# multimodallearning/stroke-prediction

Measured on AMD Instinct MI355X. Metric: train-step voxels/sec, 3D U-Net Bx2x128^3, higher is better.
Workload: dtype bf16; 1 GPU; configs[1]: U-Net 2 16 32 64 32 16 32 2, B=4/GPU, 2x128^3 -> 2x88^3, train_batch = fwd+Dice+bwd+Adam; global_batch=4, parallelism=dp1, launch=hipGraph (Learner(graph=True)), input=resident in the step's input buffers (Learner.static_batch)

## Files before the change

include/stroke_amd.h:

```cpp
#ifndef STROKE_AMD_H
#define STROKE_AMD_H

#include <stddef.h>
#include <stdint.h>

#ifdef __cplusplus
extern "C" {
#endif

typedef void* sp_stream_t;

enum { SP_OK = 0, SP_EINVAL = -1, SP_EHIP = -2 };
enum { SP_REDUCE_ROWS = 8 };
#define SP_DICE_PITCH(C) ((3 * (C) + 15) / 16 * 16)
enum { SP_VLOSS_DICE = 1, SP_VLOSS_BCE = 2 };
#define SP_VLOSS_PITCH(C) ((4 * (C) + 15) / 16 * 16)
#define SP_BLOSS_PITCH(C) SP_VLOSS_PITCH(C)
enum { SP_BF16 = 0, SP_F32 = 1,
       SP_HL = 2 };
enum { SP_ACT_NONE = 0, SP_ACT_LEAKY = 1, SP_ACT_ELU = 2, SP_ACT_SIGMOID = 3 };

int sp_version(void);
void sp_last_error(char* buf, size_t n);

typedef struct sp_bn_fin_args {
  const double* sums;
  const float* gamma;
  const float* beta;
  float* running_mean;
  float* running_var;
  float* scale;
  float* shift;
  float* mean;
  float* invstd;
  double count;
  float momentum, eps;
  int32_t nrep, training, C, CP;
} sp_bn_fin_args;

typedef struct sp_bn_bwd_args {
  const double* sums;
  const float* gamma;
  const float* mean;
  const float* invstd;
  float* dgamma;
  float* dbeta;
  float* coef;
  double count;
  float pscale;
  int32_t nrep, C, CP;
} sp_bn_bwd_args;

typedef struct sp_conv_args {
  const void* x;
  void* y;
  const void* wfrag_hi;
  const void* wfrag_lo;
  const float* in_scale;
  const float* in_shift;
  const float* bias;
  double* stats;
  const int32_t* ktab;
  int32_t dtype_in, dtype_out;
  int32_t B, Di, Hi, Wi, CPi;
  int32_t Do, Ho, Wo;
  int32_t YD, YH, YW, CPo;
  int32_t osD, osH, osW;
  int32_t ooD, ooH, ooW;
  int32_t Cout;
  int32_t sD, sH, sW;
  int32_t o0D, o0H, o0W;
  int32_t TD, TH;
  int32_t ITD, ITH, ITW;
  int32_t MT, NT;
  int32_t NTtot;
  int32_t ngroups;
  int32_t octs_per_group;
  int32_t opp;
  int32_t vsb;
  int32_t plane_bytes;
  int32_t lo_offset;
  int32_t steps_per_group;
  int32_t lds_bytes;
  int32_t act;
  float act_param;
  int32_t dma;
  int32_t zfill;
  int32_t persist;
  const void* aux;
  int32_t stats_mode;
  int32_t stats_nrep;
  int32_t ITH_zs;
  int64_t x_plane;
  void* y8;
  int64_t y8_plane;
  const float* f8_wscale;
  float y8_scale;
  int32_t f8_bin;
  int32_t group_batch;
  int32_t nslices;
  int64_t slice_wfrag_stride;
  int64_t x_lo_delta;
  int64_t y_lo_delta;
  const float* bias_tab;
  int32_t bias_tab_gstride;
  int32_t pad_;
  int64_t wfrag_gstride;
  sp_bn_bwd_args bnb;
  double* dz_sums;
  void* pool_y;
  int64_t pool_lo_delta;
  void* y2;
  int32_t split_nt, CPo2;
  int32_t pser_planes, pad2_;
} sp_conv_args;

int sp_conv3d_igemm(const sp_conv_args* a, sp_stream_t stream);
int sp_conv_prep_folded_groups(const float* w, int64_t sCo, int64_t sCi, int32_t Cout, int32_t Cin, const int32_t* kmap, int32_t nsteps,
                               int32_t NTtot, void* wfrag, int64_t frag_gstride, const float* coef, int32_t coef_gstride,
                               int32_t coef_pitch, int32_t G, const float* bias, int32_t padD, int32_t padH, int32_t padW,
                               float* bias_tab, int32_t CoutPad, sp_stream_t stream);
int sp_conv3d_igemm_multi(const sp_conv_args* args, int32_t n, sp_stream_t stream);
int sp_conv3d_par(const sp_conv_args* args, int32_t n, const void* gtab, const int32_t* gofs, const void* zeros, sp_stream_t stream);

int sp_conv3d_zm(const sp_conv_args* a, const void* zeros, sp_stream_t stream);
int sp_conv3d_zm_config(int32_t P, int32_t NT, int32_t* MT, int32_t* NSLOT, int32_t* NW);
int sp_conv3d_zm_config_ps(int32_t NT, int32_t hl, int32_t* MT, int32_t* NSLOT, int32_t* NW);

int sp_conv3d_zm_config_hl(int32_t P, int32_t NT, int32_t* MT, int32_t* NSLOT, int32_t* NW);
int sp_bn_stats_ncdhw_f32(const float* x, int32_t B, int32_t C, int64_t DHW, int32_t CP, double* sums, int32_t nrep,
                          sp_stream_t stream);
int sp_first_prep_hl(const float* w, const float* b, const float* scale, const float* shift, void* wfrag_hi, void* wfrag_lo,
                     float* bias_f, int32_t Cout, sp_stream_t stream);
int sp_first_conv_fwd_hl(const float* x, int32_t B, int32_t D, int32_t H, int32_t W, const void* wfrag_hi, const void* wfrag_lo,
                         const float* bias_f, int32_t act, float act_param, void* y, void* y_lo, double* stats, int32_t nrep,
                         int32_t Cout, sp_stream_t stream);
int sp_maxpool2_fwd_hl(const void* x, int64_t x_lo_delta, void* y, int64_t y_lo_delta, int32_t B, int32_t D, int32_t H, int32_t W,
                       int32_t CP, double* stats, sp_stream_t stream);
int sp_upsample2_crop_cat_fwd_hl(const void* low, int64_t low_lo_delta, int32_t CPu, const void* skip, int64_t skip_lo_delta, int32_t CPs,
                                 void* cat, int64_t cat_lo_delta, int32_t CPd, int32_t B, int32_t D, int32_t H, int32_t W, int32_t Ds,
                                 int32_t Hs, int32_t Ws, int64_t cat_plane, double* stats, sp_stream_t stream);
int sp_head_fwd_hl(const void* x, int64_t x_lo_delta, int64_t nvox_per_b, int32_t B, int32_t CP, int32_t C, const float* w1,
                   const float* b1, int32_t CH, const float* w2, const float* b2, int32_t NC, float slope, float* seg,
                   sp_stream_t stream);

int sp_conv3d_zm8(const sp_conv_args* a, const void* zeros, sp_stream_t stream);
int sp_conv_partial_finish(const float* partial, int32_t ngroups, int64_t nvox, int32_t CP, const float* bias ,
                           int32_t bias_stride, int32_t act, float act_param, void* y, double* stats ,
                           int32_t stats_nrep, void* y8 ,
                           int64_t y8_plane, sp_stream_t stream);
int sp_conv3d_zm8_config(int32_t P, int32_t NT, int32_t* MT, int32_t* NSLOT, int32_t* NW);
int sp_conv_prep_f8(const float* w, int64_t sCo, int64_t sCi, int32_t Cout, int32_t Cin, const int32_t* kmap,
                    int32_t nsteps, int32_t NT, void* wfrag, const float* fold_scale, const float* fold_shift,
                    int32_t ntaps, const float* bias, float* bias_out, float* winv, float out_scale, sp_stream_t stream);
typedef struct sp_f8_prep_item {
  const float* w;
  int64_t sCo, sCi;
  int32_t Cout, Cin;
  const int32_t* kmap;
  int32_t nsteps, NT;
  void* wfrag;
  const float* fold_scale;
  const float* fold_shift;
  const float* bias;
  float* bias_out;
  float* winv;
  int32_t ntaps;
  float out_scale;
} sp_f8_prep_item;
int sp_conv_prep_f8_batch(const sp_f8_prep_item* items_dev, int32_t n, int32_t max_rows, sp_stream_t stream);
int sp_quantize_f8(const void* src, int32_t CP, int64_t src_plane, void* dst, int64_t dst_plane, int64_t nvox, int32_t fmt,
                   float scale, sp_stream_t stream);

typedef struct sp_conv3d_desc {
  int32_t B, Cin, Cout, D, H, W;
  int32_t grad;
  int32_t padD, padH, padW;
  int32_t transposed;
} sp_conv3d_desc;
typedef struct sp_conv3d_plan_t {
  int32_t cin_op, cout_op;
  int32_t P, NT, MT, NW, NSLOT, KS, nsteps, ITH;
  int32_t Di, Hi, Wi, Do, Ho, Wo, o0;
  int32_t o0H, o0W, mirror;
  int64_t x_elems, y_elems;
  int64_t workspace_bytes;
  int64_t off_zero, off_ktab, off_kmap, off_bias, off_wfrag;
} sp_conv3d_plan_t;
int sp_conv3d_plan(const sp_conv3d_desc* d, sp_conv3d_plan_t* plan);
int sp_conv3d_tables(const sp_conv3d_desc* d, const sp_conv3d_plan_t* plan, int32_t* ktab, int32_t* kmap);
int sp_conv3d_init(const sp_conv3d_desc* d, const sp_conv3d_plan_t* plan, void* workspace, sp_stream_t stream);
int sp_conv3d_set_weights(const sp_conv3d_desc* d, const sp_conv3d_plan_t* plan, void* workspace, const float* w,
                          const float* bias, const float* bn_scale, const float* bn_shift, sp_stream_t stream);
int sp_conv3d_run(const sp_conv3d_desc* d, const sp_conv3d_plan_t* plan, const void* workspace, const void* x, void* y,
                  int32_t with_bias, int32_t act, float act_param, double* stats, int32_t stats_nrep, int64_t x_plane,
                  sp_stream_t stream);

typedef struct sp_conv3d_wgrad_plan_t {
  int32_t CoT, CiT, nblocks, Do, Ho, Wo;
  int64_t workspace_bytes, off_taps, off_tapsrc, off_acc;
} sp_conv3d_wgrad_plan_t;
int sp_conv3d_wgrad_plan(const sp_conv3d_desc* d, sp_conv3d_wgrad_plan_t* p);
int sp_conv3d_wgrad_init(const sp_conv3d_desc* d, const sp_conv3d_wgrad_plan_t* p, void* workspace, sp_stream_t stream);
int sp_conv3d_wgrad_run(const sp_conv3d_desc* d, const sp_conv3d_wgrad_plan_t* p, void* workspace, const void* x, const void* dz,
                        float* dw, const float* bn_scale , const float* bn_shift, const double* dbias_sums ,
                        int32_t dbias_stride, float* dbias_grad , const float* w_for_bn ,
                        double* bn_sums , int32_t bn_nrep, int64_t x_plane, sp_stream_t stream);

typedef struct sp_conv_fc_args {
  const void* x;
  void* y;
  const void* wfrag;
  const float* in_scale;
  const float* in_shift;
  const float* bias;
  double* stats;
  const void* aux;
  float* partial;
  const int32_t* taps;
  int32_t B, Di, Hi, Wi, CPi, Do, Ho, Wo, CPo, Cout;
  int32_t sD, sH, sW, o0D, o0H, o0W;
  int32_t ntap;
  int32_t act;
  float act_param;
  int32_t stats_mode, stats_nrep, dtype_out;
  int64_t x_plane;
  int32_t group_batch;
  int32_t coef_gstride;
} sp_conv_fc_args;
int sp_conv_fc_workspace(int32_t B, int32_t Do, int32_t Ho, int32_t Wo, int32_t Cout, int32_t ntap, int64_t* floats);
int sp_conv_fc(const sp_conv_fc_args* a, sp_stream_t stream);

int sp_conv_prep_weights(const float* w, int64_t sCo, int64_t sCi, int32_t Cout, int32_t Cin,
                         const int32_t* kmap, int32_t nsteps, int32_t NTtot,
                         void* wfrag_hi, void* wfrag_lo ,
                         const float* fold_scale ,
                         sp_stream_t stream);
typedef struct sp_prep_item {
  const float* w;
  int64_t sCo, sCi;
  int32_t Cout, Cin;
  const int32_t* kmap;
  int32_t nsteps, NTtot;
  void* wfrag_hi;
  void* wfrag_lo;
  const float* fold_scale;
  const float* bias;
  float* bias_out;
  int32_t bias_n, bias_pad;
} sp_prep_item;
int sp_conv_prep_weights_batch(const sp_prep_item* items_dev, int32_t n, int32_t max_blocks, sp_stream_t stream);
int sp_conv_fold_bias(const float* w, int64_t sCo, int64_t sCi, int32_t Cout, int32_t Cin, int32_t ntaps,
                      const float* bias, const float* shift, float* bias_out, int32_t CoutPad, sp_stream_t stream);
int sp_conv_prep_folded(const float* w, int64_t sCo, int64_t sCi, int32_t Cout, int32_t Cin, const int32_t* kmap,
                        int32_t nsteps, int32_t NTtot, void* wfrag_hi, void* wfrag_lo, const float* fold_scale,
                        int32_t ntaps, const float* bias, const float* fold_shift, float* bias_out, int32_t CoutPad,
                        sp_stream_t stream);

int sp_conv_prep_folded_bn(const float* w, int64_t sCo, int64_t sCi, int32_t Cout, int32_t Cin, const int32_t* kmap,
                           int32_t nsteps, int32_t NTtot, void* wfrag_hi, void* wfrag_lo, int32_t ntaps, const float* bias,
                           float* bias_out, int32_t CoutPad, const sp_bn_fin_args* bn, sp_stream_t stream);
int sp_first_prep_bn(const float* w, const float* b, void* wfrag, void* wfrag_lo, float* bias_f, int32_t Cout,
                     const sp_bn_fin_args* bn, sp_stream_t stream);

typedef struct sp_wgrad_args {
  const void* x;
  const void* dz;
  const float* in_scale;
  const float* in_shift;
  const float* dz_scale;
// ... 313 lines not shown
```

stroke-prediction_amd/csrc/sp_conv_dma.hip:

```cpp
#include "sp_common.h"

struct ConvDmaDev {
  sp_conv_args a;
  FastDiv d_itw, d_ith, d_plane;
  FastDiv d_tx, d_ty, d_tz;
  uint32_t ntx, nty, ntz, nblk;
  int32_t plane_chunks, group_chunks, nruns, log2_opp;
  int32_t row_chunks, segs_per_row, nrows, njobs;
  FastDiv d_segs, d_rows;
};

typedef __attribute__((address_space(3))) void lds_void;
typedef const __attribute__((address_space(1))) void gbl_void;


#ifdef SP_CONV_STAMPS
#define SP_NSTAMP 6
extern __device__ unsigned long long sp_stamp_buf[32768][SP_NSTAMP];
#define STAMP(k)                                                                              \
  do {                                                                                        \
    __builtin_amdgcn_sched_barrier(0);                                                        \
    unsigned long long t_;                                                                    \
    asm volatile("s_memtime %0\n\ts_waitcnt lgkmcnt(0)" : "=s"(t_)::"memory");                \
    __builtin_amdgcn_sched_barrier(0);                                                        \
    if (threadIdx.x == 0 && blockIdx.y == 0 && blockIdx.x < 32768) sp_stamp_buf[blockIdx.x][k] = t_; \
  } while (0)
#else
#define STAMP(k)
#endif

template <int NT, int MT, int KS, typename TOUT, bool HL = false>
__global__ __launch_bounds__(256, ((NT == 1 && KS > 0) ? 4 : 1)) void conv_igemm_dma_kernel(const ConvDmaDev P) {
  static_assert(!HL || KS == 0, "bf16 pairs: run-time K loop only");
  extern __shared__ __attribute__((aligned(16))) unsigned char lds[];
  const sp_conv_args& a = P.a;
  const int tid = threadIdx.x, lane = tid & 63, wave = __builtin_amdgcn_readfirstlane(tid >> 6);
  const int lv = lane & 15, lg = lane >> 4;

  uint32_t t = xcd_remap(blockIdx.x, P.nblk);
  uint32_t q = fdiv(t, P.d_tx); const int tx = t - q * P.ntx; t = q;
  q = fdiv(t, P.d_ty); const int ty = t - q * P.nty; t = q;
  q = fdiv(t, P.d_tz); const int tz = t - q * P.ntz; const int b = q;
  const int oz0 = tz * a.TD, oy0 = ty * a.TH, ox0 = tx * 16;
  const int nt0 = blockIdx.y * NT;
  const int iz0 = oz0 * a.sD + a.o0D, iy0 = oy0 * a.sH + a.o0H, ix0 = ox0 * a.sW + a.o0W;

  int* ktab_l = reinterpret_cast<int*>(lds);
  const int ktab_bytes = (a.steps_per_group * 16 + 15) & ~15;
  unsigned char* tile = lds + ktab_bytes;
  for (int i = tid; i < a.steps_per_group * 4; i += 256) ktab_l[i] = a.ktab[i];

  int vbase[MT];
#pragma unroll
  for (int m = 0; m < MT; ++m) {
    const int r = wave * MT + m;
    const int rz = r / a.TH, ry = r - rz * a.TH;
    vbase[m] = ((rz * a.sD * a.ITH + ry * a.sH) * a.ITW + lv * a.sW) * a.vsb;
  }
  f32x4 acc[NT][MT];
#pragma unroll
  for (int n = 0; n < NT; ++n)
#pragma unroll
    for (int m = 0; m < MT; ++m) acc[n][m] = f32x4{0.f, 0.f, 0.f, 0.f};

  const int xpitch = a.x_plane ? 16 : a.CPi;
  const bf16_t* __restrict__ xin = reinterpret_cast<const bf16_t*>(a.x) + (size_t)b * a.Di * a.Hi * a.Wi * xpitch;
  const bf16x8* __restrict__ wf_hi = reinterpret_cast<const bf16x8*>(a.wfrag_hi);
  const bool border = a.zfill && (iz0 < 0 || iy0 < 0 || ix0 < 0 || iz0 + a.ITD > a.Di || iy0 + a.ITH > a.Hi || ix0 + a.ITW > a.Wi);
  const int opp_mask = a.opp - 1;

  int job_goff[2], job_loff[2];
#pragma unroll
  for (int k = 0; k < 2; ++k) {
    int j = k * 64 + lane;
    j = j < P.njobs ? j : P.njobs - 1;
    const uint32_t prow = fdiv(j, P.d_segs);
    const int seg = j - prow * P.segs_per_row;
    const uint32_t pl = fdiv(prow, P.d_rows);
    const int row = prow - pl * P.nrows;
    const uint32_t vz = fdiv(row, P.d_ith);
    const int vy = row - vz * a.ITH;
    const int cz = min(max(iz0 + (int)vz, 0), a.Di - 1), cy = min(max(iy0 + vy, 0), a.Hi - 1);
    job_goff[k] = ((cz * a.Hi + cy) * a.Wi) * xpitch + (a.x_plane ? (int)pl * (int)a.x_plane : (int)pl * a.opp * 8);
    job_loff[k] = (int)pl * a.plane_bytes + row * P.row_chunks * 16 + seg * 1024 + (seg << 24);
  }
  STAMP(0);
  for (int grp = 0; grp < a.ngroups; ++grp) {
    if (grp > 0) __syncthreads();
    const int oct0 = grp * a.octs_per_group;
#pragma unroll
    for (int k = 0; k < 2; ++k) {
      const int nj = min(64, P.njobs - k * 64);
      for (int j = wave; j < nj; j += 4) {
        const int goff = __builtin_amdgcn_readlane(job_goff[k], j);
        const int lo = __builtin_amdgcn_readlane(job_loff[k], j);
        const int seg = lo >> 24;
        const int ch = seg * 64 + lane;
        if (ch < P.row_chunks) {
          const int cx = min(max(ix0 + (ch >> P.log2_opp), 0), a.Wi - 1);
          const bf16_t* src = a.x_plane ? xin + goff + (size_t)(oct0 >> 1) * a.x_plane + (cx * 16 + (ch & opp_mask) * 8)
                                        : xin + goff + (cx * a.CPi + (oct0 + (ch & opp_mask)) * 8);
#ifndef SP_NO_DMA
          sp_dma16(src, tile + (lo & 0xffffff));
          if constexpr (HL) sp_dma16(reinterpret_cast<const unsigned char*>(src) + a.x_lo_delta, tile + a.lo_offset + (lo & 0xffffff));
#endif
        }
      }
    }
    const size_t gstep0 = (size_t)grp * a.steps_per_group;
    const size_t fstride = (size_t)a.NTtot * 64;
    const bf16x8* wp = wf_hi + (gstep0 * a.NTtot + nt0) * 64 + lane;
    const bf16x8* wpl = HL ? reinterpret_cast<const bf16x8*>(a.wfrag_lo) + (gstep0 * a.NTtot + nt0) * 64 + lane : nullptr;
    bf16x8 wreg[KS > 0 ? KS : 1][NT];
    bf16x8 wa0[NT], wa1[NT];
    bf16x8 wl0[HL ? NT : 1], wl1[HL ? NT : 1], wl2[HL ? NT : 1], wl3[HL ? NT : 1];
    if (KS > 0) {
#pragma unroll
      for (int s = 0; s < KS; ++s)
#pragma unroll
        for (int n = 0; n < NT; ++n) wreg[s][n] = wp[s * fstride + (size_t)n * 64];
    } else {
#pragma unroll
      for (int n = 0; n < NT; ++n) wa0[n] = wp[(size_t)n * 64];
      if constexpr (HL) {
#pragma unroll
        for (int n = 0; n < NT; ++n) wl0[n] = wpl[(size_t)n * 64];
      }
    }
    if (grp == 0) STAMP(1);
    asm volatile("s_waitcnt vmcnt(0)" ::: "memory");
    __syncthreads();
    if (grp == 0) STAMP(2);
    if (border) {
      for (int r = wave; r < P.nruns; r += 4) {
        const int i = r * 64 + lane;
        if (i < P.group_chunks) {
          const uint32_t pl = fdiv(i, P.d_plane);
          const int ii = i - pl * P.plane_chunks;
          const uint32_t vox = (uint32_t)ii >> P.log2_opp;
          const uint32_t row = fdiv(vox, P.d_itw);
          const int vx = vox - row * a.ITW;
          const uint32_t vz = fdiv(row, P.d_ith);
          const int vy = row - vz * a.ITH;
          const int gz = iz0 + (int)vz, gy = iy0 + vy, gx = ix0 + vx;
          if (!((unsigned)gz < (unsigned)a.Di && (unsigned)gy < (unsigned)a.Hi && (unsigned)gx < (unsigned)a.Wi)) {
            *reinterpret_cast<uint4*>(tile + (size_t)i * 16) = make_uint4(0, 0, 0, 0);
            if constexpr (HL) *reinterpret_cast<uint4*>(tile + a.lo_offset + (size_t)i * 16) = make_uint4(0, 0, 0, 0);
          }
        }
      }
      __syncthreads();
    }

    bf16x8 x0[MT], x1[MT];
    bf16x8 xl0[HL ? MT : 1], xl1[HL ? MT : 1];
#define SP_LDX(dst, koff_)                                                                            \
  _Pragma("unroll") for (int m = 0; m < MT; ++m) dst[m] = *reinterpret_cast<const bf16x8*>(tile + vbase[m] + (koff_));
#define SP_LDXL(dst, koff_)                                                                           \
  if constexpr (HL) { _Pragma("unroll") for (int m = 0; m < MT; ++m) dst[m] = *reinterpret_cast<const bf16x8*>(tile + a.lo_offset + vbase[m] + (koff_)); }
#define SP_MMA(wv, xv)                                                                                \
  _Pragma("unroll") for (int m = 0; m < MT; ++m)                                                      \
      _Pragma("unroll") for (int n = 0; n < NT; ++n) acc[n][m] = SP_MFMA16(wv[n], xv[m], acc[n][m], 0, 0, 0);
#define SP_MMAL(wv, wlv, xv, xlv)                                                                     \
  if constexpr (HL) {                                                                                 \
    _Pragma("unroll") for (int m = 0; m < MT; ++m)                                                    \
        _Pragma("unroll") for (int n = 0; n < NT; ++n) {                                              \
          acc[n][m] = SP_MFMA16(wv[n], xlv[m], acc[n][m], 0, 0, 0);                                   \
          acc[n][m] = SP_MFMA16(wlv[n], xv[m], acc[n][m], 0, 0, 0);                                   \
        }                                                                                             \
  }
    {
      const int k0 = ktab_l[lg];
      SP_LDX(x0, k0)
      SP_LDXL(xl0, k0)
    }
    if (KS > 0) {
#pragma unroll
      for (int s = 0; s < KS; ++s) {
        if (s + 1 < KS) {
          const int kn = ktab_l[(s + 1) * 4 + lg];
          if ((s & 1) == 0) { SP_LDX(x1, kn) } else { SP_LDX(x0, kn) }
        }
        if ((s & 1) == 0) { SP_MMA(wreg[s], x0) } else { SP_MMA(wreg[s], x1) }
      }
    } else {
      const int nst = a.steps_per_group;
      bf16x8 wa2[NT], wa3[NT];
#define SP_LDW(dst, dstl, step_)                                                                      \
  { const int st_ = (step_) < nst ? (step_) : nst - 1;                                                \
    _Pragma("unroll") for (int n = 0; n < NT; ++n) dst[n] = wp[(size_t)st_ * fstride + (size_t)n * 64]; \
    if constexpr (HL) { _Pragma("unroll") for (int n = 0; n < NT; ++n) dstl[n] = wpl[(size_t)st_ * fstride + (size_t)n * 64]; } }
      SP_LDW(wa1, wl1, 1)
      SP_LDW(wa2, wl2, 2)
      for (int s = 0; s < nst; s += 4) {
        SP_LDW(wa3, wl3, s + 3)
        { const int kn = ktab_l[(s + 1) * 4 + lg]; SP_LDX(x1, kn) SP_LDXL(xl1, kn) }
        SP_MMA(wa0, x0)
        SP_MMAL(wa0, wl0, x0, xl0)
        SP_LDW(wa0, wl0, s + 4)
        if (s + 2 < nst) { const int kn = ktab_l[(s + 2) * 4 + lg]; SP_LDX(x0, kn) SP_LDXL(xl0, kn) }
        SP_MMA(wa1, x1)
        SP_MMAL(wa1, wl1, x1, xl1)
        if (s + 2 < nst) {
          SP_LDW(wa1, wl1, s + 5)
          { const int kn = ktab_l[(s + 3) * 4 + lg]; SP_LDX(x1, kn) SP_LDXL(xl1, kn) }
          SP_MMA(wa2, x0)
          SP_MMAL(wa2, wl2, x0, xl0)
          SP_LDW(wa2, wl2, s + 6)
          if (s + 4 < nst) { const int kn = ktab_l[(s + 4) * 4 + lg]; SP_LDX(x0, kn) SP_LDXL(xl0, kn) }
          SP_MMA(wa3, x1)
          SP_MMAL(wa3, wl3, x1, xl1)
        }
      }
#undef SP_LDW
    }
#undef SP_LDX
#undef SP_LDXL
#undef SP_MMA
#undef SP_MMAL
  }

  STAMP(3);
  TOUT* __restrict__ yout = reinterpret_cast<TOUT*>(a.y) + (size_t)b * a.YD * a.YH * a.YW * a.CPo;
  const int ox = ox0 + lv;
  int obase[MT];
#pragma unroll
  for (int m = 0; m < MT; ++m) {
    const int r = wave * MT + m;
    const int rz = r / a.TH, ry = r - rz * a.TH;
    const int oz = oz0 + rz, oy = oy0 + ry;
    const bool valid = oz < a.Do && oy < a.Ho && ox < a.Wo;
    obase[m] = valid ? (((oz * a.osD + a.ooD) * a.YH + (oy * a.osH + a.ooH)) * a.YW + (ox * a.osW + a.ooW)) * a.CPo : -1;
  }
  float s1[NT][4], s2[NT][4];
#pragma unroll
  for (int n = 0; n < NT; ++n) {
    const int c0 = (nt0 + n) * 16 + lg * 4;
    float bj[4] = {0.f, 0.f, 0.f, 0.f};
    if (a.bias) { const float4 bb = *reinterpret_cast<const float4*>(a.bias + c0); bj[0] = bb.x; bj[1] = bb.y; bj[2] = bb.z; bj[3] = bb.w; }
#pragma unroll
    for (int j = 0; j < 4; ++j) s1[n][j] = s2[n][j] = 0.f;
    const bool cok = c0 < a.CPo;
    const bool full = c0 + 4 <= a.Cout;
    const bool lin = full && (a.act == SP_ACT_LEAKY || a.act == SP_ACT_NONE);
    const float slope = a.act == SP_ACT_LEAKY ? a.act_param : 1.f;
    const bool want_stats = a.stats != nullptr;
#pragma unroll
    for (int m = 0; m < MT; ++m) {
      float v[4];
      if (lin) {
#pragma unroll
        for (int j = 0; j < 4; ++j) { const float z = acc[n][m][j] + bj[j]; v[j] = fmaxf(z, slope * z); }
      } else {
#pragma unroll
        for (int j = 0; j < 4; ++j) {
          const float z = act_fwd(a.act, a.act_param, acc[n][m][j] + bj[j]);
          v[j] = (c0 + j < a.Cout) ? z : 0.f;
        }
      }
      if (obase[m] >= 0 && cok) {
#ifdef SP_NO_STORE
        if (v[0] == 123456.f)
#endif
        if constexpr (HL) sp_hl_st4(yout + (size_t)obase[m] + c0, a.y_lo_delta, v);
        else Store<TOUT>::st4(yout + (size_t)obase[m] + c0, v);
        if (want_stats) {
          if (sizeof(TOUT) == 2 && !HL) {
#pragma unroll
            for (int j = 0; j < 4; ++j) v[j] = bf2f(f2bf(v[j]));
          }
          if (a.stats_mode == 1) {
            float xv[4] = {0.f, 0.f, 0.f, 0.f};
            if constexpr (!HL) Store<TOUT>::ld4(reinterpret_cast<const TOUT*>(a.aux) + (size_t)b * a.YD * a.YH * a.YW * a.CPo + (size_t)obase[m] + c0, xv);
#pragma unroll
            for (int j = 0; j < 4; ++j) { s1[n][j] += v[j]; s2[n][j] = fmaf(v[j], xv[j], s2[n][j]); }
          } else {
#pragma unroll
            for (int j = 0; j < 4; ++j) { s1[n][j] += v[j]; s2[n][j] = fmaf(v[j], v[j], s2[n][j]); }
          }
        }
      }
    }
  }
  STAMP(4);
  if (a.stats) {
    __syncthreads();
    float* red = reinterpret_cast<float*>(lds);
#pragma unroll
    for (int n = 0; n < NT; ++n)
#pragma unroll
      for (int j = 0; j < 4; ++j) {
        const float x1 = row16_sum(s1[n][j]), x2 = row16_sum(s2[n][j]);
        if (lv == 0) {
          red[wave * (NT * 32) + (n * 16 + lg * 4 + j) * 2] = x1;
          red[wave * (NT * 32) + (n * 16 + lg * 4 + j) * 2 + 1] = x2;
        }
      }
    __syncthreads();
    double* const g_stats = a.stats + (size_t)(a.group_batch > 0 ? b / a.group_batch : 0) * a.stats_nrep * a.CPo * 2;
    for (int i = tid; i < NT * 16 * 2; i += 256) {
      const int c = nt0 * 16 + (i >> 1);
      if (c < a.CPo) atomicAdd(&g_stats[(size_t)(blockIdx.x & (a.stats_nrep - 1)) * a.CPo * 2 + (size_t)c * 2 + (i & 1)], (double)sp_cols_sum(red, NT * 32, 4, i));
    }
  }
  STAMP(5);
}

struct ConvZsDev {
  sp_conv_args a;
  int32_t ITH, ITW, S, nchunks, ZC, nzc, nty, ntx;
  uint32_t ncols;
  FastDiv d_itw, d_tx, d_ty, d_zc;
};

template <int NT, int MT, int KS, typename TOUT>
__global__ __launch_bounds__(256, (NT == 1 ? 2 : 1)) void conv_igemm_zs_kernel(const ConvZsDev P) {
  extern __shared__ __attribute__((aligned(16))) unsigned char lds[];
  constexpr int NJ = 5;
  const sp_conv_args& a = P.a;
  const int tid = threadIdx.x, lane = tid & 63, wave = __builtin_amdgcn_readfirstlane(tid >> 6);
  const int lv = lane & 15, lg = lane >> 4;
  unsigned char* ring = lds;

  int kv[KS];
#pragma unroll
  for (int s = 0; s < KS; ++s) kv[s] = a.ktab[s * 4 + lg];
  int vbase[MT];
#pragma unroll
  for (int m = 0; m < MT; ++m) vbase[m] = ((wave * MT + m) * P.ITW + lv) * 32;
  const bf16x8* __restrict__ wf_hi = reinterpret_cast<const bf16x8*>(a.wfrag_hi);
  bf16x8 wreg[KS][NT];
#pragma unroll
  for (int s = 0; s < KS; ++s)
#pragma unroll
    for (int n = 0; n < NT; ++n) wreg[s][n] = wf_hi[((size_t)s * a.NTtot + n) * 64 + lane];

  uint32_t rel[NJ];
  int crd[NJ];
#pragma unroll
  for (int j = 0; j < NJ; ++j) {
    const int c = (wave + 4 * j) * 64 + lane;
    const int cc = c < P.nchunks ? c : P.nchunks - 1;
    const int half = cc & 1, vox = cc >> 1;
    const int vy = fdiv(vox, P.d_itw), vx = vox - vy * P.ITW;
    rel[j] = (uint32_t)(((vy * a.Wi + vx) * a.CPi + half * 8) * 2);
    crd[j] = vy | (vx << 8) | (c < P.nchunks ? 0 : (1 << 30));
  }
  float bj[NT][4], s1[NT][4], s2[NT][4];
#pragma unroll
  for (int n = 0; n < NT; ++n)
#pragma unroll
    for (int j = 0; j < 4; ++j) { bj[n][j] = a.bias ? a.bias[n * 16 + lg * 4 + j] : 0.f; s1[n][j] = s2[n][j] = 0.f; }
  const bool linact = a.act == SP_ACT_LEAKY || a.act == SP_ACT_NONE;
  const float slope = a.act == SP_ACT_LEAKY ? a.act_param : 1.f;
  const bool want_stats = a.stats != nullptr;

  const uint32_t vb = xcd_remap(blockIdx.x, gridDim.x);
  const uint64_t T = (uint64_t)P.ncols * a.Do;
  uint64_t pos = T * vb / gridDim.x;
  const uint64_t pend = T * (vb + 1) / gridDim.x;
  while (pos < pend) {
    const uint32_t col = (uint32_t)(pos / (uint32_t)a.Do);
    const int z0 = (int)(pos - (uint64_t)col * a.Do);
    const int z1 = (int)min((uint64_t)a.Do, (uint64_t)z0 + (pend - pos));
    pos += (uint64_t)(z1 - z0);
    uint32_t t = col;
    uint32_t q = fdiv(t, P.d_tx); const int tx = t - q * P.ntx; t = q;
    q = fdiv(t, P.d_ty); const int ty = t - q * P.nty; const int b = q;
    const int oy0 = ty * (4 * MT), ox0 = tx * 16;
    const int iy0 = oy0 + a.o0H, ix0 = ox0 + a.o0W;
    const bf16_t* xin = reinterpret_cast<const bf16_t*>(a.x) + (size_t)b * a.Di * a.Hi * a.Wi * a.CPi;
    int vmask = 0;
#pragma unroll
    for (int j = 0; j < NJ; ++j) {
      const int vy = crd[j] & 0xff, vx = (crd[j] >> 8) & 0xff;
      if (!(crd[j] >> 30) && (unsigned)(iy0 + vy) < (unsigned)a.Hi && (unsigned)(ix0 + vx) < (unsigned)a.Wi) vmask |= 1 << j;
    }
    auto load_plane = [&](int iz, int slot) {
      unsigned char* dst0 = ring + slot * P.S;
      const bool zin = (unsigned)iz < (unsigned)a.Di;
      const unsigned char* src0 = reinterpret_cast<const unsigned char*>(xin) + (((int64_t)iz * a.Hi + iy0) * a.Wi + ix0) * a.CPi * 2;
#pragma unroll
      for (int j = 0; j < NJ; ++j) {
        unsigned char* dst = dst0 + (wave + 4 * j) * 1024;
        if (!(crd[j] >> 30)) {
          if (zin && ((vmask >> j) & 1)) sp_dma16(src0 + rel[j], dst);
          else *reinterpret_cast<uint4*>(dst + lane * 16) = make_uint4(0, 0, 0, 0);
        }
      }
    };
    __syncthreads();
    load_plane(z0 + a.o0D, 0);
    load_plane(z0 + a.o0D + 1, 1);
    load_plane(z0 + a.o0D + 2, 2);
    asm volatile("s_waitcnt vmcnt(0)" ::: "memory");
    __syncthreads();
    TOUT* __restrict__ yout = reinterpret_cast<TOUT*>(a.y) + (size_t)b * a.YD * a.YH * a.YW * a.CPo;
    const int ox = ox0 + lv;
    for (int z = z0; z < z1; ++z) {
      const int sl = (z - z0) & 3;
      if (z + 1 < z1) load_plane(z + a.o0D + 3, (sl + 3) & 3);
      f32x4 acc[NT][MT];
#pragma unroll
      for (int n = 0; n < NT; ++n)
#pragma unroll
        for (int m = 0; m < MT; ++m) acc[n][m] = f32x4{0.f, 0.f, 0.f, 0.f};
      bf16x8 x0[MT], x1[MT];
#define ZS_OFF(s_) ((((sl + (kv[s_] & 3)) & 3) * P.S) + (kv[s_] & ~15))
      {
        const int k0 = ZS_OFF(0);
#pragma unroll
        for (int m = 0; m < MT; ++m) x0[m] = *reinterpret_cast<const bf16x8*>(ring + vbase[m] + k0);
      }
#pragma unroll
      for (int s = 0; s < KS; ++s) {
        if (s + 1 < KS) {
          const int kn = ZS_OFF(s + 1 < KS ? s + 1 : s);
          if ((s & 1) == 0) {
#pragma unroll
            for (int m = 0; m < MT; ++m) x1[m] = *reinterpret_cast<const bf16x8*>(ring + vbase[m] + kn);
          } else {
#pragma unroll
            for (int m = 0; m < MT; ++m) x0[m] = *reinterpret_cast<const bf16x8*>(ring + vbase[m] + kn);
          }
        }
        if ((s & 1) == 0) {
#pragma unroll
          for (int m = 0; m < MT; ++m)
#pragma unroll
            for (int n = 0; n < NT; ++n) acc[n][m] = SP_MFMA16(wreg[s][n], x0[m], acc[n][m], 0, 0, 0);
        } else {
#pragma unroll
          for (int m = 0; m < MT; ++m)
#pragma unroll
            for (int n = 0; n < NT; ++n) acc[n][m] = SP_MFMA16(wreg[s][n], x1[m], acc[n][m], 0, 0, 0);
        }
      }
#undef ZS_OFF
#pragma unroll
      for (int m = 0; m < MT; ++m) {
        const int oy = oy0 + wave * MT + m;
        const bool inside = oy < a.Ho && ox < a.Wo;
        const size_t vo = (size_t)((((z * a.osD + a.ooD) * a.YH + (oy * a.osH + a.ooH)) * a.YW + (ox * a.osW + a.ooW)) * a.CPo);
#pragma unroll
        for (int n = 0; n < NT; ++n) {
          const int c0 = n * 16 + lg * 4;
          const bool lin = linact && (c0 + 4 <= a.Cout);
          float v[4];
          if (lin) {
#pragma unroll
            for (int j = 0; j < 4; ++j) { const float zz = acc[n][m][j] + bj[n][j]; v[j] = fmaxf(zz, slope * zz); }
          } else {
#pragma unroll
            for (int j = 0; j < 4; ++j) {
              const float zz = act_fwd(a.act, a.act_param, acc[n][m][j] + bj[n][j]);
              v[j] = (c0 + j < a.Cout) ? zz : 0.f;
            }
          }
          if (inside && c0 < a.CPo) {
            Store<TOUT>::st4(yout + vo + c0, v);
            if (want_stats) {
              if (sizeof(TOUT) == 2) {
#pragma unroll
                for (int j = 0; j < 4; ++j) v[j] = bf2f(f2bf(v[j]));
              }
#pragma unroll
              for (int j = 0; j < 4; ++j) { s1[n][j] += v[j]; s2[n][j] = fmaf(v[j], v[j], s2[n][j]); }
            }
          }
        }
      }
#ifndef SP_ZS_NOWAIT
      asm volatile("s_waitcnt vmcnt(0)" ::: "memory");
#endif
      __syncthreads();
    }
  }
  if (want_stats) {
    __syncthreads();
    float* red = reinterpret_cast<float*>(lds);
#pragma unroll
    for (int n = 0; n < NT; ++n)
#pragma unroll
      for (int j = 0; j < 4; ++j) {
        const float x1s = row16_sum(s1[n][j]), x2s = row16_sum(s2[n][j]);
        if (lv == 0) { red[wave * (NT * 32) + (n * 16 + lg * 4 + j) * 2] = x1s; red[wave * (NT * 32) + (n * 16 + lg * 4 + j) * 2 + 1] = x2s; }
      }
    __syncthreads();
    for (int i = tid; i < NT * 32; i += 256) {
      const int c = i >> 1;
      if (c < a.CPo) atomicAdd(&a.stats[(size_t)(blockIdx.x & (a.stats_nrep - 1)) * a.CPo * 2 + (size_t)c * 2 + (i & 1)], (double)sp_cols_sum(red, NT * 32, 4, i));
    }
  }
}

static int launch_zs(const sp_conv_args* a, hipStream_t st) {
  SP_CHECK_ARG(a->NT == a->NTtot && a->NT >= 1 && a->NT <= 3 && a->ngroups == 1 && a->opp == 2 && a->vsb == 32 && a->octs_per_group == 2,
               "sp_conv3d_igemm(zs): one 16-channel plane in, up to three 16-channel tiles out");
  SP_CHECK_ARG(a->sD == 1 && a->sH == 1 && a->sW == 1 && a->stats_mode == 0 && a->in_scale == nullptr && a->dtype_in == SP_BF16,
               "sp_conv3d_igemm(zs): stride 1, plain statistics, bf16 input without affine on load");
  SP_CHECK_ARG(a->steps_per_group == 14 || (a->steps_per_group == 7 && a->NT == 1), "sp_conv3d_igemm(zs): 14 (or 7) resident K steps");
  ConvZsDev P;
  P.a = *a;
  const int MT = a->NT == 3 ? 4 : 8;
  P.ITH = 4 * MT + (a->ITH_zs - 32); P.ITW = a->ITW;
  SP_CHECK_ARG(a->ITH_zs >= 32 && a->ITH_zs <= 40 && P.ITW >= 16 && P.ITW <= 24, "sp_conv3d_igemm(zs): plane extent");
  P.S = P.ITH * P.ITW * 32;
  P.nchunks = P.ITH * P.ITW * 2;
  SP_CHECK_ARG(P.nchunks <= 5 * 256 && 4 * P.S <= 160 * 1024, "sp_conv3d_igemm(zs): plane does not fit the per-lane plan");
  P.ntx = (a->Wo + 15) / 16; P.nty = (a->Ho + 4 * MT - 1) / (4 * MT);
  const int cols_xy = a->B * P.nty * P.ntx;
  const int slots = a->NT == 1 ? 512 : 256;
  P.nzc = 1; P.ZC = a->Do;
  P.ncols = (uint32_t)cols_xy;
  P.d_itw = make_fastdiv(P.ITW); P.d_tx = make_fastdiv(P.ntx); P.d_ty = make_fastdiv(P.nty); P.d_zc = make_fastdiv(P.nzc);
  const int lds_bytes = 4 * P.S;
  const uint64_t planes = (uint64_t)cols_xy * a->Do;
  const unsigned grid = planes / 4 < (uint64_t)slots ? (unsigned)(planes / 4 > 0 ? planes / 4 : 1) : (unsigned)slots;
#define SP_ZS(N_, M_, K_, T_)                                                                                        \
  {                                                                                                                  \
    auto kern = conv_igemm_zs_kernel<N_, M_, K_, T_>;                                                                \
    SP_ENSURE_LDS(kern, lds_bytes, "sp_conv");                                                                       \
    hipLaunchKernelGGL(kern, dim3(grid), dim3(256), lds_bytes, st, P);                                               \
  }
#define SP_ZS_T(N_, M_, K_) { if (a->dtype_out == SP_F32) SP_ZS(N_, M_, K_, float) else SP_ZS(N_, M_, K_, bf16_t) }
  if (a->NT == 1 && a->steps_per_group == 14) SP_ZS_T(1, 8, 14)
  else if (a->NT == 1) SP_ZS_T(1, 8, 7)
  else if (a->NT == 2) SP_ZS_T(2, 8, 14)
  else SP_ZS_T(3, 4, 14)
#undef SP_ZS_T
#undef SP_ZS
  SP_CHECK_LAUNCH("sp_conv3d_igemm(zs)");
  return SP_OK;
}

template <int NT, int MT, int KS, typename TOUT>
static int launch_dma(const ConvDmaDev& P, dim3 grid, hipStream_t st) {
  auto kern = conv_igemm_dma_kernel<NT, MT, KS, TOUT>;
  SP_ENSURE_LDS(kern, P.a.lds_bytes, "sp_conv3d_igemm");
  hipLaunchKernelGGL(kern, grid, dim3(256), P.a.lds_bytes, st, P);
  SP_CHECK_LAUNCH("sp_conv3d_igemm(dma)");
  return SP_OK;
}

template <int NT, int MT, int KS>
static int launch_out(const ConvDmaDev& P, dim3 grid, hipStream_t st) {
  if (P.a.dtype_out == SP_F32) return launch_dma<NT, MT, KS, float>(P, grid, st);
  return launch_dma<NT, MT, KS, bf16_t>(P, grid, st);
}
template <int NT, int MT>
static int launch_hl(const ConvDmaDev& P, dim3 grid, hipStream_t st) {
  auto kern = conv_igemm_dma_kernel<NT, MT, 0, sp_hl_t, true>;
  SP_ENSURE_LDS(kern, P.a.lds_bytes, "sp_conv3d_igemm");
  hipLaunchKernelGGL(kern, grid, dim3(256), P.a.lds_bytes, st, P);
  SP_CHECK_LAUNCH("sp_conv3d_igemm(dma, pairs)");
  return SP_OK;
}

template <int NT, int MT>
static int dispatch_dma(const ConvDmaDev& P, dim3 grid, hipStream_t st) {
  const int ks = P.a.steps_per_group;
#define SP_KS(K_) if (ks == K_ && K_ * NT <= 16) return launch_out<NT, MT, (K_ * NT <= 16 ? K_ : 0)>(P, grid, st)
  SP_KS(1); SP_KS(2); SP_KS(4); SP_KS(7); SP_KS(14);
#undef SP_KS
  if (ks % 2 != 0) { sp_set_error("sp_conv3d_igemm(dma): run-time K loop needs an even step count (got %d)", ks); return SP_EINVAL; }
  return launch_out<NT, MT, 0>(P, grid, st);
}

int sp_conv3d_igemm_dma(const sp_conv_args* a, sp_stream_t stream) {
  const bool hl = a->dtype_in == SP_HL;
  SP_CHECK_ARG((a->dtype_in == SP_BF16 || hl) && a->in_scale == nullptr, "sp_conv3d_igemm(dma): needs bf16 (or bf16-pair) input and no affine on load");
  SP_CHECK_ARG(!hl || (a->dtype_out == SP_HL && a->wfrag_lo && a->lo_offset > 0 && a->x_lo_delta != 0 && a->y_lo_delta != 0 && a->persist == 0 &&
                       a->steps_per_group % 2 == 0 && a->stats_mode == 0 && a->group_batch == 0),
               "sp_conv3d_igemm(dma): bf16 pairs need lo fragments, lo tile offset, lo deltas of x and y, an even step count, the tiled kernel");
  SP_CHECK_ARG(a->group_batch == 0 || (a->persist == 0 && a->group_batch > 0 && a->B % a->group_batch == 0),
               "sp_conv3d_igemm(dma): BatchNorm groups (group_batch %d, B %d) need the tiled kernel (persist 0) and whole groups", a->group_batch, a->B);
  if (a->persist == 3) return launch_zs(a, reinterpret_cast<hipStream_t>(stream));
  SP_CHECK_ARG(a->x_plane == 0 || (a->opp == 2 && a->x_plane < (1ll << 31)), "sp_conv3d_igemm(dma): plane-major input needs 16-channel planes");
  SP_CHECK_ARG(a->opp == 1 || a->opp == 2, "sp_conv3d_igemm(dma): octets per plane must be 1 or 2");
  SP_CHECK_ARG(a->vsb == a->opp * 16 && a->plane_bytes == a->ITD * a->ITH * a->ITW * a->vsb, "sp_conv3d_igemm(dma): planes must be lane-linear (no padding)");
  SP_CHECK_ARG(a->octs_per_group % a->opp == 0, "sp_conv3d_igemm(dma): group does not consist of whole planes");
  ConvDmaDev P;
  P.a = *a;
  P.log2_opp = a->opp == 2 ? 1 : 0;
  P.plane_chunks = a->ITD * a->ITH * a->ITW * a->opp;
  P.group_chunks = P.plane_chunks * (a->octs_per_group / a->opp);
  P.nruns = (P.group_chunks + 63) / 64;
  P.row_chunks = a->ITW * a->opp;
  P.segs_per_row = (P.row_chunks + 63) / 64;
  P.nrows = a->ITD * a->ITH;
  P.njobs = (a->octs_per_group / a->opp) * P.nrows * P.segs_per_row;
  SP_CHECK_ARG(P.njobs <= 128, "sp_conv3d_igemm(dma): %d DMA jobs per group (max 128)", P.njobs);
  P.d_segs = make_fastdiv(P.segs_per_row);
  P.d_rows = make_fastdiv(P.nrows);
  const long need = ((a->steps_per_group * 16 + 15) & ~15) + (hl ? a->lo_offset + (long)P.group_chunks * 16 : (long)P.nruns * 1024);
  SP_CHECK_ARG(!hl || a->lo_offset >= (long)P.group_chunks * 16, "sp_conv3d_igemm(dma): lo tile offset %d inside the hi tile (%ld bytes)", a->lo_offset, (long)P.group_chunks * 16);
  SP_CHECK_ARG(need <= a->lds_bytes && a->lds_bytes <= 160 * 1024, "sp_conv3d_igemm(dma): LDS plan too small (need %ld, have %d)", need, a->lds_bytes);
  P.d_itw = make_fastdiv(a->ITW);
  P.d_ith = make_fastdiv(a->ITH);
  P.d_plane = make_fastdiv(P.plane_chunks);
  P.ntx = (a->Wo + 15) / 16;
  P.nty = (a->Ho + a->TH - 1) / a->TH;
  P.ntz = (a->Do + a->TD - 1) / a->TD;
  P.d_tx = make_fastdiv(P.ntx);
  P.d_ty = make_fastdiv(P.nty);
  P.d_tz = make_fastdiv(P.ntz);
  const uint64_t nblk = (uint64_t)P.ntx * P.nty * P.ntz * a->B;
  SP_CHECK_ARG(nblk < (1ull << 31), "sp_conv3d_igemm(dma): grid too large");
  P.nblk = (uint32_t)nblk;
  dim3 grid(P.nblk, a->NTtot / a->NT);
  hipStream_t st = reinterpret_cast<hipStream_t>(stream);
  if (hl) {
#define SP_CASE_HL(NT_, MT_) if (a->NT == NT_ && a->MT == MT_) return launch_hl<NT_, MT_>(P, grid, st)
    SP_CASE_HL(1, 8); SP_CASE_HL(2, 8); SP_CASE_HL(4, 8); SP_CASE_HL(1, 4); SP_CASE_HL(2, 4); SP_CASE_HL(4, 4); SP_CASE_HL(2, 2); SP_CASE_HL(4, 2);
#undef SP_CASE_HL
    sp_set_error("sp_conv3d_igemm(dma): no bf16-pair kernel for NT=%d MT=%d", a->NT, a->MT);
    return SP_EINVAL;
  }
#define SP_CASE(NT_, MT_) if (a->NT == NT_ && a->MT == MT_) return dispatch_dma<NT_, MT_>(P, grid, st)
  SP_CASE(1, 8); SP_CASE(2, 8); SP_CASE(3, 8); SP_CASE(4, 8);
  SP_CASE(1, 4); SP_CASE(2, 4); SP_CASE(3, 4); SP_CASE(4, 4);
  SP_CASE(1, 2); SP_CASE(2, 2); SP_CASE(3, 2); SP_CASE(4, 2);
#undef SP_CASE
  sp_set_error("sp_conv3d_igemm(dma): no kernel for NT=%d MT=%d", a->NT, a->MT);
  return SP_EINVAL;
}
```

Measured before the change: 3.039 billion voxels/s.

## Add intra-block split-K for DMA implicit-GEMM conv when grid underfills CUs

Adds an SK=2 variant of the DMA conv kernel that launches 512 threads per block. Two groups of four waves each take half of the run-time K loop, and the partial accumulators are then summed through LDS before the epilogue. A heuristic turns it on for bf16 MT=4, NT=2/4 layers with at least 8 non-resident K steps whose block count is below twice the CU count, and an environment variable can override it. This is meant to raise occupancy on small deep layers, at the cost of extra LDS traffic, a block-wide barrier, and half the waves sitting idle during the epilogue.

```diff
diff --git a/include/stroke_amd.h b/include/stroke_amd.h
--- a/include/stroke_amd.h
+++ b/include/stroke_amd.h
@@ -116,6 +116,7 @@
 } sp_conv_args;
 
 int sp_conv3d_igemm(const sp_conv_args* a, sp_stream_t stream);
+int sp_conv3d_igemm_splitk(const sp_conv_args* a, int32_t ncu);
 int sp_conv_prep_folded_groups(const float* w, int64_t sCo, int64_t sCi, int32_t Cout, int32_t Cin, const int32_t* kmap, int32_t nsteps,
                                int32_t NTtot, void* wfrag, int64_t frag_gstride, const float* coef, int32_t coef_gstride,
                                int32_t coef_pitch, int32_t G, const float* bias, int32_t padD, int32_t padH, int32_t padW,
diff --git a/stroke-prediction_amd/csrc/sp_conv_dma.hip b/stroke-prediction_amd/csrc/sp_conv_dma.hip
--- a/stroke-prediction_amd/csrc/sp_conv_dma.hip
+++ b/stroke-prediction_amd/csrc/sp_conv_dma.hip
@@ -1,3 +1,4 @@
+#include <stdlib.h>
 #include "sp_common.h"
 
 struct ConvDmaDev {
@@ -29,12 +30,15 @@
 #define STAMP(k)
 #endif
 
-template <int NT, int MT, int KS, typename TOUT, bool HL = false>
-__global__ __launch_bounds__(256, ((NT == 1 && KS > 0) ? 4 : 1)) void conv_igemm_dma_kernel(const ConvDmaDev P) {
+template <int NT, int MT, int KS, typename TOUT, bool HL = false, int SK = 1>
+__global__ __launch_bounds__(256 * SK, ((NT == 1 && KS > 0) ? 4 : 1)) void conv_igemm_dma_kernel(const ConvDmaDev P) {
   static_assert(!HL || KS == 0, "bf16 pairs: run-time K loop only");
+  static_assert(SK == 1 || (SK == 2 && KS == 0 && !HL), "split K: two halves of the run-time K loop, bf16");
+  constexpr int NW = 4 * SK, NTHR = 256 * SK;
   extern __shared__ __attribute__((aligned(16))) unsigned char lds[];
   const sp_conv_args& a = P.a;
-  const int tid = threadIdx.x, lane = tid & 63, wave = __builtin_amdgcn_readfirstlane(tid >> 6);
+  const int tid = threadIdx.x, lane = tid & 63, wave_id = __builtin_amdgcn_readfirstlane(tid >> 6);
+  const int wave = SK == 2 ? wave_id & 3 : wave_id, khalf = SK == 2 ? wave_id >> 2 : 0;
   const int lv = lane & 15, lg = lane >> 4;
 
   uint32_t t = xcd_remap(blockIdx.x, P.nblk);
@@ -48,7 +52,7 @@
   int* ktab_l = reinterpret_cast<int*>(lds);
   const int ktab_bytes = (a.steps_per_group * 16 + 15) & ~15;
   unsigned char* tile = lds + ktab_bytes;
-  for (int i = tid; i < a.steps_per_group * 4; i += 256) ktab_l[i] = a.ktab[i];
+  for (int i = tid; i < a.steps_per_group * 4; i += NTHR) ktab_l[i] = a.ktab[i];
 
   int vbase[MT];
 #pragma unroll
@@ -68,6 +72,12 @@
   const bf16x8* __restrict__ wf_hi = reinterpret_cast<const bf16x8*>(a.wfrag_hi);
   const bool border = a.zfill && (iz0 < 0 || iy0 < 0 || ix0 < 0 || iz0 + a.ITD > a.Di || iy0 + a.ITH > a.Hi || ix0 + a.ITW > a.Wi);
   const int opp_mask = a.opp - 1;
+  int kstep0 = 0, nst = a.steps_per_group;
+  if constexpr (SK == 2) {
+    const int h = ((nst >> 1) + 1) & ~1;
+    kstep0 = khalf ? h : 0;
+    nst = khalf ? nst - h : h;
+  }
 
   int job_goff[2], job_loff[2];
 #pragma unroll
@@ -91,7 +101,7 @@
 #pragma unroll
     for (int k = 0; k < 2; ++k) {
       const int nj = min(64, P.njobs - k * 64);
-      for (int j = wave; j < nj; j += 4) {
+      for (int j = wave_id; j < nj; j += NW) {
         const int goff = __builtin_amdgcn_readlane(job_goff[k], j);
         const int lo = __builtin_amdgcn_readlane(job_loff[k], j);
         const int seg = lo >> 24;
@@ -107,7 +117,7 @@
         }
       }
     }
-    const size_t gstep0 = (size_t)grp * a.steps_per_group;
+    const size_t gstep0 = (size_t)grp * a.steps_per_group + kstep0;
     const size_t fstride = (size_t)a.NTtot * 64;
     const bf16x8* wp = wf_hi + (gstep0 * a.NTtot + nt0) * 64 + lane;
     const bf16x8* wpl = HL ? reinterpret_cast<const bf16x8*>(a.wfrag_lo) + (gstep0 * a.NTtot + nt0) * 64 + lane : nullptr;
@@ -132,7 +142,7 @@
     __syncthreads();
     if (grp == 0) STAMP(2);
     if (border) {
-      for (int r = wave; r < P.nruns; r += 4) {
+      for (int r = wave_id; r < P.nruns; r += NW) {
         const int i = r * 64 + lane;
         if (i < P.group_chunks) {
           const uint32_t pl = fdiv(i, P.d_plane);
@@ -169,8 +179,9 @@
           acc[n][m] = SP_MFMA16(wlv[n], xv[m], acc[n][m], 0, 0, 0);                                   \
         }                                                                                             \
   }
+    const int* kt = ktab_l + kstep0 * 4;
     {
-      const int k0 = ktab_l[lg];
+      const int k0 = kt[lg];
       SP_LDX(x0, k0)
       SP_LDXL(xl0, k0)
     }
@@ -178,13 +189,12 @@
 #pragma unroll
       for (int s = 0; s < KS; ++s) {
         if (s + 1 < KS) {
-          const int kn = ktab_l[(s + 1) * 4 + lg];
+          const int kn = kt[(s + 1) * 4 + lg];
           if ((s & 1) == 0) { SP_LDX(x1, kn) } else { SP_LDX(x0, kn) }
         }
         if ((s & 1) == 0) { SP_MMA(wreg[s], x0) } else { SP_MMA(wreg[s], x1) }
       }
     } else {
-      const int nst = a.steps_per_group;
       bf16x8 wa2[NT], wa3[NT];
 #define SP_LDW(dst, dstl, step_)                                                                      \
   { const int st_ = (step_) < nst ? (step_) : nst - 1;                                                \
@@ -194,20 +204,20 @@
       SP_LDW(wa2, wl2, 2)
       for (int s = 0; s < nst; s += 4) {
         SP_LDW(wa3, wl3, s + 3)
-        { const int kn = ktab_l[(s + 1) * 4 + lg]; SP_LDX(x1, kn) SP_LDXL(xl1, kn) }
+        { const int kn = kt[(s + 1) * 4 + lg]; SP_LDX(x1, kn) SP_LDXL(xl1, kn) }
         SP_MMA(wa0, x0)
         SP_MMAL(wa0, wl0, x0, xl0)
         SP_LDW(wa0, wl0, s + 4)
-        if (s + 2 < nst) { const int kn = ktab_l[(s + 2) * 4 + lg]; SP_LDX(x0, kn) SP_LDXL(xl0, kn) }
+        if (s + 2 < nst) { const int kn = kt[(s + 2) * 4 + lg]; SP_LDX(x0, kn) SP_LDXL(xl0, kn) }
         SP_MMA(wa1, x1)
         SP_MMAL(wa1, wl1, x1, xl1)
         if (s + 2 < nst) {
           SP_LDW(wa1, wl1, s + 5)
-          { const int kn = ktab_l[(s + 3) * 4 + lg]; SP_LDX(x1, kn) SP_LDXL(xl1, kn) }
+          { const int kn = kt[(s + 3) * 4 + lg]; SP_LDX(x1, kn) SP_LDXL(xl1, kn) }
           SP_MMA(wa2, x0)
           SP_MMAL(wa2, wl2, x0, xl0)
           SP_LDW(wa2, wl2, s + 6)
-          if (s + 4 < nst) { const int kn = ktab_l[(s + 4) * 4 + lg]; SP_LDX(x0, kn) SP_LDXL(xl0, kn) }
+          if (s + 4 < nst) { const int kn = kt[(s + 4) * 4 + lg]; SP_LDX(x0, kn) SP_LDXL(xl0, kn) }
           SP_MMA(wa3, x1)
           SP_MMAL(wa3, wl3, x1, xl1)
         }
@@ -220,6 +230,23 @@
 #undef SP_MMAL
   }
 
+  if constexpr (SK == 2) {
+    __syncthreads();
+    f32x4* part = reinterpret_cast<f32x4*>(lds) + (tid & 255);
+    if (khalf) {
+#pragma unroll
+      for (int n = 0; n < NT; ++n)
+#pragma unroll
+        for (int m = 0; m < MT; ++m) part[(n * MT + m) * 256] = acc[n][m];
+    }
+    __syncthreads();
+    if (!khalf) {
+#pragma unroll
+      for (int n = 0; n < NT; ++n)
+#pragma unroll
+        for (int m = 0; m < MT; ++m) acc[n][m] += part[(n * MT + m) * 256];
+    }
+  }
   STAMP(3);
   TOUT* __restrict__ yout = reinterpret_cast<TOUT*>(a.y) + (size_t)b * a.YD * a.YH * a.YW * a.CPo;
   const int ox = ox0 + lv;
@@ -229,7 +256,7 @@
     const int r = wave * MT + m;
     const int rz = r / a.TH, ry = r - rz * a.TH;
     const int oz = oz0 + rz, oy = oy0 + ry;
-    const bool valid = oz < a.Do && oy < a.Ho && ox < a.Wo;
+    const bool valid = oz < a.Do && oy < a.Ho && ox < a.Wo && !khalf;
     obase[m] = valid ? (((oz * a.osD + a.ooD) * a.YH + (oy * a.osH + a.ooH)) * a.YW + (ox * a.osW + a.ooW)) * a.CPo : -1;
   }
   float s1[NT][4], s2[NT][4];
@@ -291,14 +318,14 @@
 #pragma unroll
       for (int j = 0; j < 4; ++j) {
         const float x1 = row16_sum(s1[n][j]), x2 = row16_sum(s2[n][j]);
-        if (lv == 0) {
+        if (lv == 0 && !khalf) {
           red[wave * (NT * 32) + (n * 16 + lg * 4 + j) * 2] = x1;
           red[wave * (NT * 32) + (n * 16 + lg * 4 + j) * 2 + 1] = x2;
         }
       }
     __syncthreads();
     double* const g_stats = a.stats + (size_t)(a.group_batch > 0 ? b / a.group_batch : 0) * a.stats_nrep * a.CPo * 2;
-    for (int i = tid; i < NT * 16 * 2; i += 256) {
+    for (int i = tid; i < NT * 16 * 2; i += NTHR) {
       const int c = nt0 * 16 + (i >> 1);
       if (c < a.CPo) atomicAdd(&g_stats[(size_t)(blockIdx.x & (a.stats_nrep - 1)) * a.CPo * 2 + (size_t)c * 2 + (i & 1)], (double)sp_cols_sum(red, NT * 32, 4, i));
     }
@@ -558,8 +585,41 @@
 }
 
 template <int NT, int MT>
+static int launch_sk2(const ConvDmaDev& P, dim3 grid, hipStream_t st) {
+  auto kern = conv_igemm_dma_kernel<NT, MT, 0, bf16_t, false, 2>;
+  const int lds_bytes = P.a.lds_bytes > NT * MT * 4096 ? P.a.lds_bytes : NT * MT * 4096;
+  SP_ENSURE_LDS(kern, lds_bytes, "sp_conv3d_igemm");
+  hipLaunchKernelGGL(kern, grid, dim3(512), lds_bytes, st, P);
+  SP_CHECK_LAUNCH("sp_conv3d_igemm(dma, split K)");
+  return SP_OK;
+}
+
+extern "C" int sp_conv3d_igemm_splitk(const sp_conv_args* a, int32_t ncu) {
+  if (!a->dma || a->persist != 0 || a->dtype_in != SP_BF16 || a->dtype_out != SP_BF16) return 1;
+  if (!(a->MT == 4 && (a->NT == 4 || a->NT == 2)) || a->NT <= 0 || a->TD <= 0 || a->TH <= 0) return 1;
+  const int ks = a->steps_per_group;
+  const bool resident = (ks == 1 || ks == 2 || ks == 4 || ks == 7 || ks == 14) && ks * a->NT <= 16;
+  if (resident || ks % 2 != 0 || ks < 8) return 1;
+  const int64_t nblk = (int64_t)((a->Wo + 15) / 16) * ((a->Ho + a->TH - 1) / a->TH) * ((a->Do + a->TD - 1) / a->TD) * a->B;
+  return nblk * (a->NTtot / a->NT) < 2 * (int64_t)ncu ? 2 : 1;
+}
+
+static int device_cu_count() {
+  static int ncu[64];
+  int dev = 0;
+  if (hipGetDevice(&dev) != hipSuccess || dev < 0 || dev >= 64) return 0;
+  if (ncu[dev] == 0 && hipDeviceGetAttribute(&ncu[dev], hipDeviceAttributeMultiprocessorCount, dev) != hipSuccess) ncu[dev] = 0;
+  return ncu[dev];
+}
+
+template <int NT, int MT>
 static int dispatch_dma(const ConvDmaDev& P, dim3 grid, hipStream_t st) {
   const int ks = P.a.steps_per_group;
+  if constexpr (MT == 4 && (NT == 4 || NT == 2)) {
+    const char* knob = getenv("SP_CONV_SPLITK");
+    const int mode = knob ? atoi(knob) : 1;
+    if (mode != 0 && sp_conv3d_igemm_splitk(&P.a, mode == 2 ? (1 << 28) : device_cu_count()) == 2) return launch_sk2<NT, MT>(P, grid, st);
+  }
 #define SP_KS(K_) if (ks == K_ && K_ * NT <= 16) return launch_out<NT, MT, (K_ * NT <= 16 ? K_ : 0)>(P, grid, st)
   SP_KS(1); SP_KS(2); SP_KS(4); SP_KS(7); SP_KS(14);
 #undef SP_KS
```

Result: slower. 2.999 billion voxels/s (-1.3%).
